# meyer-lab/cmtf-pls

Hardware: AMD Instinct MI355X
Metric: nipals_iters_per_sec (higher is better)
Workload: dtype f32

## Files before the change

cmtf_pls_amd/csrc/rank1.hip:

```cpp
#include "common.hpp"
#include <atomic>

namespace cmtfpls {

constexpr int kTile = 16;
constexpr int kMaxTiles = 256;
constexpr int kMaxSteps = 48;

struct Rank1Ctl {
  int done;
  int final_buf;
  int steps_used;
  int last_step;
  double pad[6];
};
__host__ __device__ __forceinline__ size_t rank1_ctl_bytes(int nt) {
  return sizeof(Rank1Ctl) + ((size_t)(kMaxSteps + 2) * nt + 2 * (size_t)nt * nt) * sizeof(double);
}
__device__ __forceinline__ double* ctl_trace(Rank1Ctl* c, int nt, int step) { return reinterpret_cast<double*>(c + 1) + (size_t)step * nt; }
__device__ __forceinline__ double* ctl_fro(Rank1Ctl* c, int nt, int which) {
  return reinterpret_cast<double*>(c + 1) + (size_t)(kMaxSteps + 2) * nt + (size_t)which * nt * nt;
}

__device__ __forceinline__ double pow2_scale_from_trace(const double* parts, int nt, double* tr_out) {
// ... 6 lines not shown
  return ldexp(1.0, -e);
}

typedef double d4r_t __attribute__((ext_vector_type(4)));

__global__ __launch_bounds__(kTile* kTile) void syrk_step_kernel(const double* __restrict__ M, int n, int k, int ld,
                                                                double* __restrict__ C, Rank1Ctl* __restrict__ ctl,
                                                                int step, int out_buf, double* __restrict__ C_keep) {
  __shared__ double red[4][kTile * kTile];
  __shared__ double diag[kTile];
  __shared__ double s_scale;
  __shared__ int s_done;
  __shared__ double fsum[4];
  __shared__ double tr_s[kMaxTiles];
  const int tx = threadIdx.x, ty = threadIdx.y, tid = ty * kTile + tx;
  const int lane = tid & 63, wv = tid >> 6, ri = lane & 15, kq = lane >> 4;
  const int nt = (n + kTile - 1) / kTile;
  const int i0 = blockIdx.y * kTile, j0 = blockIdx.x * kTile;

  constexpr int KC = 128, KW = 8;
  const bool ra = (i0 + ri) < n, rb = (j0 + ri) < n;
  const double* __restrict__ rowa = M + (int64_t)(ra ? i0 + ri : 0) * ld;
  const double* __restrict__ rowb = M + (int64_t)(rb ? j0 + ri : 0) * ld;
  const int cl = 32 * wv + KW * kq;
  double a[KW], b[KW];
#pragma unroll
  for (int s2 = 0; s2 < KW; ++s2) {
    const int c = cl + s2;
    const int cc = (c < k) ? c : 0;
    a[s2] = rowa[cc];
    b[s2] = rowb[cc];
  }

  double fro_in = 0.0;
  if (step >= 1) {
    int zero = 0;
    asm volatile("" : "+v"(zero));
    const int last_in = (&ctl->last_step)[zero];
    const int done_in = (&ctl->done)[zero] | ((last_in >= 0 && last_in < step) ? 1 : 0);
    const double* fp = ctl_fro(ctl, nt, (step - 1) & 1);
    const double trv = ctl_trace(ctl, nt, step - 1)[(tid < nt) ? tid : 0];
    double f = fp[(tid < nt * nt) ? tid : 0];
    if (tid < nt) tr_s[tid] = trv;
    if (tid >= nt * nt) f = 0.0;
    for (int i = tid + kTile * kTile; i < nt * nt; i += kTile * kTile) f += fp[i];
    f = wave_sum(f);
    if ((tid & 63) == 0) fsum[tid >> 6] = f;
    if (tid == 0) s_done = done_in;
    __syncthreads();
    fro_in = ((fsum[0] + fsum[1]) + fsum[2]) + fsum[3];
  }
  if (tid == 0) {
    int done = 0;
    double scale = 1.0;
    if (step == 0) {
      if (blockIdx.x == 0 && blockIdx.y == 0) { ctl->done = 0; ctl->final_buf = -1; ctl->steps_used = 0; ctl->last_step = -1; }
    } else {
      done = s_done;
      if (!done) {
        double tr1;
        scale = pow2_scale_from_trace(tr_s, nt, &tr1);
        const double rho = fro_in / (tr1 * tr1);
        const bool rank_one_in = !(tr1 > 0.0) || rho >= 1.0 - 1e-13;
        const bool rank_one_out = rho >= 1.0 - 1e-7;
        if (blockIdx.x == 0 && blockIdx.y == 0) {
          if (rank_one_in) { ctl->done = 1; ctl->final_buf = out_buf ^ 1; }
          else {
            ctl->steps_used = step;
            if (rank_one_out) { ctl->last_step = step; ctl->final_buf = out_buf; }
          }
        }
        if (rank_one_in) done = 1;
      }
    }
    s_scale = scale;
    s_done = done;
  }
  __syncthreads();
  if (s_done) return;
  const double scale = s_scale;

  d4r_t acc = d4r_t{0.0, 0.0, 0.0, 0.0};
  for (int kk = 0; kk < k; kk += KC) {
    if (kk > 0) {
#pragma unroll
      for (int s2 = 0; s2 < KW; ++s2) {
        const int c = kk + cl + s2;
        const int cc = (c < k) ? c : 0;
        a[s2] = rowa[cc];
        b[s2] = rowb[cc];
      }
    }
#pragma unroll
    for (int s2 = 0; s2 < KW; ++s2) {
      const bool cok = (kk + cl + s2) < k;
      const double av = (ra && cok) ? a[s2] : 0.0;
      const double bv = (rb && cok) ? b[s2] : 0.0;
      acc = __builtin_amdgcn_mfma_f64_16x16x4f64(av, bv, acc, 0, 0, 0);
    }
  }
#pragma unroll
  for (int e = 0; e < 4; ++e) red[wv][(kq + 4 * e) * kTile + ri] = acc[e];
  __syncthreads();
  double cacc = ((red[0][tid] + red[1][tid]) + red[2][tid]) + red[3][tid];
  cacc *= scale * scale;
  const bool inside = (i0 + ty < n && j0 + tx < n);
  if (inside) C[(int64_t)(i0 + ty) * n + (j0 + tx)] = cacc;
  if (inside && C_keep) C_keep[(int64_t)(i0 + ty) * n + (j0 + tx)] = cacc;
  {
    double sq = inside ? cacc * cacc : 0.0;
    sq = wave_sum(sq);
    if ((tid & 63) == 0) fsum[tid >> 6] = sq;
    __syncthreads();
    if (tid == 0) ctl_fro(ctl, nt, step & 1)[blockIdx.y * nt + blockIdx.x] = ((fsum[0] + fsum[1]) + fsum[2]) + fsum[3];
  }
  if (blockIdx.x == blockIdx.y) {
    if (tx == ty) diag[tx] = (i0 + ty < n) ? cacc : 0.0;
    __syncthreads();
    if (tid == 0) {
      double t = 0.0;
      for (int l = 0; l < kTile; ++l) t += diag[l];
      ctl_trace(ctl, nt, step)[blockIdx.x] = t;
    }
  }
}

constexpr unsigned long long kChainEmpty = ~0ull;
constexpr int kChainMaxSteps = 31;
constexpr int kChainSpin = 1 << 15;

__device__ __forceinline__ double chain_ld(const double* p) {
  return __longlong_as_double((long long)__hip_atomic_load(reinterpret_cast<const unsigned long long*>(p), __ATOMIC_RELAXED, __HIP_MEMORY_SCOPE_AGENT));
}
__device__ __forceinline__ void chain_st(double* p, double v) {
  unsigned long long b = (unsigned long long)__double_as_longlong(v);
  if (b == kChainEmpty) b = 0x7FF8000000000000ull;
  __hip_atomic_store(reinterpret_cast<unsigned long long*>(p), b, __ATOMIC_RELAXED, __HIP_MEMORY_SCOPE_AGENT);
}
__device__ __forceinline__ bool chain_empty(double v) { return (unsigned long long)__double_as_longlong(v) == kChainEmpty; }

__global__ __launch_bounds__(256) void chain_preset_kernel(unsigned long long* __restrict__ p, int64_t n) {
  for (int64_t i = (int64_t)blockIdx.x * 256 + threadIdx.x; i < n; i += (int64_t)gridDim.x * 256) p[i] = kChainEmpty;
}

#ifdef CMTFPLS_CHAIN_PROFILE
__device__ unsigned long long g_chain_prof[1024];
#define CHAIN_STAMP(slot) do { if (first_wg && tid == 0 && step < 32) g_chain_prof[step * 8 + (slot)] = __builtin_amdgcn_s_memrealtime(); } while (0)
#define CHAIN_COUNT(slot, v) do { if (first_wg && tid == 0 && step < 32) g_chain_prof[step * 8 + (slot)] = (unsigned long long)(v); } while (0)
#else
#define CHAIN_STAMP(slot) do { } while (0)
#define CHAIN_COUNT(slot, v) do { } while (0)
#endif

__global__ __launch_bounds__(kTile* kTile) void syrk_chain_kernel(const double* __restrict__ M0, int n, int k0,
                                                                 double* gbufs, double* trs, double* fros, double* gave_up,
                                                                 Rank1Ctl* __restrict__ ctl, int n_squarings) {
  constexpr int KC = 128, KW = 8, LDP = KC + 2;
  __shared__ __attribute__((aligned(16))) double pan[2][kTile][LDP];
  __shared__ double red[2][4][kTile * kTile];
  __shared__ double diag[2][kTile];
  __shared__ double fsum[2][4];
  __shared__ double cfro[2][4];
  __shared__ double ctr[2][kTile];
  __shared__ int cdead[2];
  const int tx = threadIdx.x, ty = threadIdx.y, tid = ty * kTile + tx;
  const int lane = tid & 63, wv = tid >> 6, ri = lane & 15, kq = lane >> 4;
  const int nt = (n + kTile - 1) / kTile, nt2 = nt * nt;
  const int i0 = blockIdx.y * kTile, j0 = blockIdx.x * kTile;
  const bool first_wg = blockIdx.x == 0 && blockIdx.y == 0;
  const bool ra = (i0 + ri) < n, rb = (j0 + ri) < n;
  const int cl = 32 * wv + KW * kq;
  const int64_t nn = (int64_t)n * n;
  const double qnan = __longlong_as_double(0x7FF8000000000000ll);
  bool dead = false;
  if (first_wg && tid == 0) { ctl->done = 0; ctl->final_buf = -1; ctl->steps_used = 0; ctl->last_step = -1; }
  if (tid < 2) cdead[tid] = 0;
  int last_step = -1;
  for (int step = 0; step <= n_squarings; ++step) {
    if (last_step >= 0) break;
    const int par = step & 1;
    const double* __restrict__ M = step == 0 ? M0 : gbufs + (int64_t)(step - 1) * nn;
    const int k = step == 0 ? k0 : n, ld = k;
    double* C = gbufs + (int64_t)step * nn;
    double a[KW], b[KW];
    double scale = 1.0;
    bool input_is_result = false;
    d4r_t acc = d4r_t{0.0, 0.0, 0.0, 0.0};
    CHAIN_STAMP(0);
    for (int kk = 0; kk < k; kk += KC) {
      if (step == 0) {
        const double* __restrict__ rowa = M + (int64_t)(ra ? i0 + ri : 0) * ld;
        const double* __restrict__ rowb = M + (int64_t)(rb ? j0 + ri : 0) * ld;
#pragma unroll
        for (int s2 = 0; s2 < KW; ++s2) {
          const int c = kk + cl + s2;
          const int cc = (c < k) ? c : 0;
          a[s2] = rowa[cc];
          b[s2] = rowb[cc];
        }
      } else {
        double va[8], vb[8], trv = 0.0, f = 0.0;
        const bool first_chunk = kk == 0;
        const double* tp = trs + (int64_t)(step - 1) * nt;
        const double* fp = fros + (int64_t)(step - 1) * nt2;
        unsigned offa[8], offb[8];
#pragma unroll
        for (int i = 0; i < 8; ++i) {
          const int e = tid + 256 * i, r = e >> 7, c = kk + (e & 127);
          const int cc = (c < k) ? c : 0;
          const int rra = (i0 + r < n) ? i0 + r : 0, rrb = (j0 + r < n) ? j0 + r : 0;
          offa[i] = (unsigned)(rra * ld + cc);
          offb[i] = (unsigned)(rrb * ld + cc);
        }
        int spins = 0;
        for (;;) {
          bool ok = true;
#pragma unroll
          for (int i = 0; i < 8; ++i) {
            va[i] = chain_ld(M + offa[i]);
            vb[i] = chain_ld(M + offb[i]);
          }
          if (first_chunk) {
            f = chain_ld(fp + ((tid < nt2) ? tid : 0));
            ok = !chain_empty(f);
            if (wv == 0) {
              trv = chain_ld(tp + ((lane < nt) ? lane : 0));
              ok = ok && !chain_empty(trv);
            }
          }
#pragma unroll
          for (int i = 0; i < 8; ++i) ok = ok && !chain_empty(va[i]) && !chain_empty(vb[i]);
          if (dead || __all(ok)) break;
          if (++spins > kChainSpin) {
            dead = true;
            if (lane == 0) chain_st(gave_up, 1.0);
            break;
          }
        }
        CHAIN_STAMP(1);
        CHAIN_COUNT(7, spins);
        if (kk > 0) __syncthreads();
#pragma unroll
        for (int i = 0; i < 8; ++i) {
          const int e = tid + 256 * i, r = e >> 7, c = e & 127;
          pan[0][r][c] = dead ? qnan : va[i];
          pan[1][r][c] = dead ? qnan : vb[i];
        }
        if (first_chunk) {
          const double fw = wave_sum((tid < nt2) ? f : 0.0);
          if (lane == 0) cfro[par][wv] = fw;
          if (wv == 0 && lane < nt) ctr[par][lane] = trv;
          if (dead && lane == 0) cdead[par] = 1;
        }
        __syncthreads();
        CHAIN_STAMP(2);
        if (first_chunk) {
          const double fro_in = ((cfro[par][0] + cfro[par][1]) + cfro[par][2]) + cfro[par][3];
          double tr1 = 0.0;
          for (int i = 0; i < nt; ++i) tr1 += ctr[par][i];
          if ((tr1 > 0.0) && isfinite(tr1)) {
            int e;
            frexp(tr1, &e);
            scale = ldexp(1.0, -e);
          }
          const bool gone = cdead[par] != 0;
          const double rho = fro_in / (tr1 * tr1);
          const bool rank_one_in = !gone && (!(tr1 > 0.0) || rho >= 1.0 - 1e-13);
          const bool rank_one_out = !gone && rho >= 1.0 - 1e-7;
          if (first_wg && tid == 0) {
            if (rank_one_in) { ctl->done = 1; ctl->final_buf = step - 1; }
            else {
              ctl->steps_used = step;
              if (rank_one_out) { ctl->last_step = step; ctl->final_buf = step; }
            }
          }
          if (rank_one_in) { input_is_result = true; break; }
          if (rank_one_out) last_step = step;
        }
#pragma unroll
        for (int s2 = 0; s2 < KW; ++s2) {
          a[s2] = pan[0][ri][cl + s2];
          b[s2] = pan[1][ri][cl + s2];
        }
      }
#pragma unroll
      for (int s2 = 0; s2 < KW; ++s2) {
        const bool cok = (kk + cl + s2) < k;
        const double av = (ra && cok) ? a[s2] : 0.0;
        const double bv = (rb && cok) ? b[s2] : 0.0;
        acc = __builtin_amdgcn_mfma_f64_16x16x4f64(av, bv, acc, 0, 0, 0);
      }
    }
    if (input_is_result) break;
    CHAIN_STAMP(3);
#pragma unroll
    for (int e = 0; e < 4; ++e) red[par][wv][(kq + 4 * e) * kTile + ri] = acc[e];
    __syncthreads();
    CHAIN_STAMP(4);
    double cacc = ((red[par][0][tid] + red[par][1][tid]) + red[par][2][tid]) + red[par][3][tid];
    cacc *= scale * scale;
    const bool inside = (i0 + ty < n && j0 + tx < n);
    if (inside) chain_st(C + (int64_t)(i0 + ty) * n + (j0 + tx), cacc);
    CHAIN_STAMP(5);
    double sq = inside ? cacc * cacc : 0.0;
    sq = wave_sum(sq);
    if ((tid & 63) == 0) fsum[par][tid >> 6] = sq;
    if (blockIdx.x == blockIdx.y && tx == ty) diag[par][tx] = (i0 + ty < n) ? cacc : 0.0;
    __syncthreads();
    if (tid == 0) {
      chain_st(fros + (int64_t)step * nt2 + blockIdx.y * nt + blockIdx.x, ((fsum[par][0] + fsum[par][1]) + fsum[par][2]) + fsum[par][3]);
      if (blockIdx.x == blockIdx.y) {
        double t = 0.0;
        for (int l = 0; l < kTile; ++l) t += diag[par][l];
        chain_st(trs + (int64_t)step * nt + blockIdx.x, t);
      }
    }
    CHAIN_STAMP(6);
  }
}

__global__ __launch_bounds__(256) void transpose_kernel(const double* __restrict__ Z, int A, int B, double* __restrict__ Zt) {
  const int64_t idx = (int64_t)blockIdx.x * 256 + threadIdx.x;
  if (idx >= (int64_t)A * B) return;
  const int b = (int)(idx / A), a = (int)(idx % A);
  Zt[idx] = Z[(int64_t)a * B + b];
}

__global__ __launch_bounds__(256) void rank1_seed_xy_kernel(const double* __restrict__ M, int n, int k,
                                                           const double* __restrict__ gbase, int64_t gstride,
                                                           const double* __restrict__ G0,
                                                           const Rank1Ctl* __restrict__ ctl, int last_buf, int ny_blocks,
                                                           double* __restrict__ y, double* __restrict__ x) {
  extern __shared__ double seed[];
  __shared__ double red[16];
  __shared__ double rsum[8][33];
  __shared__ double bestv[4];
  __shared__ int besti[4];
  const int fb = (ctl->final_buf >= 0) ? ctl->final_buf : last_buf;
  const double* G = gbase + (int64_t)fb * gstride;
  double bv = -1.0;
  int bi = 0;
  for (int i = threadIdx.x; i < n; i += 256) {
    const double d = G[(int64_t)i * n + i];
    if (d > bv) { bv = d; bi = i; }
  }
#pragma unroll
  for (int m = 32; m > 0; m >>= 1) {
    const double ov = __shfl_xor(bv, m, 64);
    const int oi = __shfl_xor(bi, m, 64);
    if (ov > bv || (ov == bv && oi < bi)) { bv = ov; bi = oi; }
  }
  if ((threadIdx.x & 63) == 0) { bestv[threadIdx.x >> 6] = bv; besti[threadIdx.x >> 6] = bi; }
  __syncthreads();
  bv = bestv[0];
  bi = besti[0];
  for (int w = 1; w < 4; ++w)
    if (bestv[w] > bv || (bestv[w] == bv && besti[w] < bi)) { bv = bestv[w]; bi = besti[w]; }
  double ss = 0.0;
  for (int i = threadIdx.x; i < n; i += 256) {
    const double g = G[(int64_t)bi * n + i];
    seed[i] = g;
    ss = fma(g, g, ss);
  }
  const double nrm = sqrt(block_sum(ss, red));
  for (int i = threadIdx.x; i < n; i += 256) seed[i] = seed[i] / nrm;
  __syncthreads();
  if ((int)blockIdx.x >= ny_blocks) {
    const int j = ((int)blockIdx.x - ny_blocks) * 4 + (threadIdx.x >> 6);
    const int lane = threadIdx.x & 63;
    if (j < n) {
      double s = 0.0;
      for (int i = lane; i < n; i += 64) s = fma(G0[(int64_t)j * n + i], seed[i], s);
      s = wave_sum(s);
      if (lane == 0) x[j] = s;
    }
    return;
  }
  const int cx = threadIdx.x & 31, ry = threadIdx.x >> 5;
  const int c = blockIdx.x * 32 + cx;
  double s = 0.0;
  if (c < k)
    for (int j = ry; j < n; j += 8) s = fma(M[(int64_t)j * k + c], seed[j], s);
  rsum[ry][cx] = s;
  __syncthreads();
  if (ry == 0 && c < k) {
    double tot = 0.0;
#pragma unroll
    for (int g = 0; g < 8; ++g) tot += rsum[g][cx];
    y[c] = tot;
  }
}

__device__ __forceinline__ void rank1_write_info(double* __restrict__ info, const Rank1Ctl* __restrict__ ctl, const double* gave) {
  if (!info) return;
  if (gave && !chain_empty(chain_ld(gave))) { info[0] = 0.0; info[1] = -1.0; return; }
  info[0] = (ctl->done || ctl->last_step >= 0) ? 1.0 : 0.0;
  info[1] = (double)ctl->steps_used;
}

__device__ __forceinline__ void rank1_final_body(const double* x, const double* y,
                                                 int n, int k, int x_is_A, const Rank1Ctl* __restrict__ ctl,
                                                 double* __restrict__ wA, double* __restrict__ wB,
                                                 double* __restrict__ sigma, double* __restrict__ info, const double* gave) {
  __shared__ double red[2][16];
  __shared__ double bestv[16];
  __shared__ int besti[16];
  double sx = 0.0, sy = 0.0;
  for (int i = threadIdx.x; i < n; i += 1024) sx = fma(x[i], x[i], sx);
  for (int i = threadIdx.x; i < k; i += 1024) sy = fma(y[i], y[i], sy);
  const double nx = sqrt(block_sum(sx, red[0]));
  const double ny = sqrt(block_sum(sy, red[1]));
  const double* vb = x_is_A ? y : x;
  const int nb = x_is_A ? k : n;
  double bv = -1.0;
  int bi = 0;
  for (int i = threadIdx.x; i < nb; i += 1024) {
    const double d = fabs(vb[i]);
    if (d > bv) { bv = d; bi = i; }
  }
#pragma unroll
  for (int m = 32; m > 0; m >>= 1) {
    const double ov = __shfl_xor(bv, m, 64);
    const int oi = __shfl_xor(bi, m, 64);
    if (ov > bv || (ov == bv && oi < bi)) { bv = ov; bi = oi; }
  }
  if ((threadIdx.x & 63) == 0) { bestv[threadIdx.x >> 6] = bv; besti[threadIdx.x >> 6] = bi; }
  __syncthreads();
  bv = bestv[0];
  bi = besti[0];
  for (int w = 1; w < 16; ++w)
    if (bestv[w] > bv || (bestv[w] == bv && besti[w] < bi)) { bv = bestv[w]; bi = besti[w]; }
  const bool gv = gave && !chain_empty(chain_ld(gave));
  const double sgn = gv ? __longlong_as_double(0x7FF8000000000000ll) : ((vb[bi] < 0.0) ? -1.0 : 1.0);
  double* ox = x_is_A ? wA : wB;
  double* oy = x_is_A ? wB : wA;
  for (int i = threadIdx.x; i < n; i += 1024) ox[i] = sgn * (x[i] / nx);
  for (int i = threadIdx.x; i < k; i += 1024) oy[i] = sgn * (y[i] / ny);
  if (threadIdx.x == 0) {
    if (sigma) sigma[0] = nx / ny;
    rank1_write_info(info, ctl, gave);
  }
}

__global__ __launch_bounds__(1024) void rank1_final_kernel(const double* __restrict__ x, const double* __restrict__ y,
                                                          int n, int k, int x_is_A, const Rank1Ctl* __restrict__ ctl,
                                                          double* __restrict__ wA, double* __restrict__ wB,
                                                          double* __restrict__ sigma, double* __restrict__ info, const double* gave) {
  rank1_final_body(x, y, n, k, x_is_A, ctl, wA, wB, sigma, info, gave);
}

__global__ __launch_bounds__(1024) void rank1_final_score_kernel(const double* __restrict__ x, const double* __restrict__ y,
                                                                int n, int k, int x_is_A, const Rank1Ctl* __restrict__ ctl,
                                                                double* __restrict__ wA, double* __restrict__ wB,
                                                                double* __restrict__ info, const double* __restrict__ S, int A, int B,
                                                                double* __restrict__ t, const double* gave) {
  extern __shared__ double lds[];
  __shared__ double red[2][16];
  __shared__ double bestv[16];
  __shared__ int besti[16];
  double* sA = lds;
  double* sB = lds + ((A + 1) & ~1);
  double sx = 0.0, sy = 0.0;
  for (int i = threadIdx.x; i < n; i += 1024) sx = fma(x[i], x[i], sx);
  for (int i = threadIdx.x; i < k; i += 1024) sy = fma(y[i], y[i], sy);
  const double nx = sqrt(block_sum(sx, red[0]));
  const double ny = sqrt(block_sum(sy, red[1]));
  const double* vb = x_is_A ? y : x;
  const int nb = x_is_A ? k : n;
  double bv = -1.0;
  int bi = 0;
  for (int i = threadIdx.x; i < nb; i += 1024) {
    const double d = fabs(vb[i]);
    if (d > bv) { bv = d; bi = i; }
  }
#pragma unroll
  for (int m = 32; m > 0; m >>= 1) {
    const double ov = __shfl_xor(bv, m, 64);
    const int oi = __shfl_xor(bi, m, 64);
    if (ov > bv || (ov == bv && oi < bi)) { bv = ov; bi = oi; }
  }
  if ((threadIdx.x & 63) == 0) { bestv[threadIdx.x >> 6] = bv; besti[threadIdx.x >> 6] = bi; }
  __syncthreads();
  bv = bestv[0];
  bi = besti[0];
  for (int w = 1; w < 16; ++w)
    if (bestv[w] > bv || (bestv[w] == bv && besti[w] < bi)) { bv = bestv[w]; bi = besti[w]; }
  const bool gv = gave && !chain_empty(chain_ld(gave));
  const double sgn = gv ? __longlong_as_double(0x7FF8000000000000ll) : ((vb[bi] < 0.0) ? -1.0 : 1.0);
  double* lx = x_is_A ? sA : sB;
  double* ly = x_is_A ? sB : sA;
  double* ox = x_is_A ? wA : wB;
  double* oy = x_is_A ? wB : wA;
  const bool store = blockIdx.x == 0;
  for (int i = threadIdx.x; i < n; i += 1024) {
    const double v = sgn * (x[i] / nx);
    lx[i] = v;
    if (store) ox[i] = v;
  }
  for (int i = threadIdx.x; i < k; i += 1024) {
    const double v = sgn * (y[i] / ny);
    ly[i] = v;
    if (store) oy[i] = v;
  }
  if (store && threadIdx.x == 0) rank1_write_info(info, ctl, gave);
  __syncthreads();
  using VT = Pack<double, 2>;
  const int64_t P = (int64_t)A * B;
  const int64_t step = (int64_t)1024 * 2;
  const double* __restrict__ xr = S + (int64_t)blockIdx.x * P;
  KronWalk w((int64_t)threadIdx.x * 2, step, B);
  double acc = 0.0;
  int64_t c = (int64_t)threadIdx.x * 2;
  constexpr int UN = 4;
  for (; c + (UN - 1) * step < P; c += UN * step) {
    VT xs[UN];
#pragma unroll
    for (int u = 0; u < UN; ++u) xs[u] = ld_stream(reinterpret_cast<const VT*>(xr + c + u * step));
#pragma unroll
    for (int u = 0; u < UN; ++u) {
      double d = 0.0;
      d = fma(xs[u].e[0], sB[w.k], d);
      d = fma(xs[u].e[1], sB[w.k + 1], d);
      acc = fma(sA[w.j], d, acc);
      w.next();
    }
  }
  for (; c < P; c += step) {
    const VT xv = ld_stream(reinterpret_cast<const VT*>(xr + c));
    double d = 0.0;
    d = fma(xv.e[0], sB[w.k], d);
    d = fma(xv.e[1], sB[w.k + 1], d);
    acc = fma(sA[w.j], d, acc);
    w.next();
  }
  acc = block_sum(acc, red[0]);
  if (threadIdx.x == 0) t[blockIdx.x] = acc;
}

static inline size_t align_up(size_t x, size_t a) { return (x + a - 1) / a * a; }

static std::atomic<int> g_chain_on{1};

static int chain_slots() {
  static int slots = 0;
  if (slots == 0) {
    int dev = 0, cus = 0;
    if (hipGetDevice(&dev) != hipSuccess || hipDeviceGetAttribute(&cus, hipDeviceAttributeMultiprocessorCount, dev) != hipSuccess || cus <= 0) cus = 256;
    slots = 2 * cus;
  }
  return slots;
}

}

using namespace cmtfpls;

extern "C" {

size_t cmtfpls_rank1_workspace_bytes(int A, int B) {
  if (A <= 0 || B <= 0) return 0;
  const size_t n = (size_t)(A < B ? A : B), k = (size_t)(A < B ? B : A);
  const size_t nt = (n + kTile - 1) / kTile;
  const size_t chain = nt * nt <= 256 ? align_up(((size_t)(kChainMaxSteps + 1) * (n * n + nt + nt * nt) + 1) * sizeof(double), 256) : 0;
  return align_up(rank1_ctl_bytes((int)nt), 256) + 3 * align_up(n * n * sizeof(double), 256) +
         align_up((size_t)A * B * sizeof(double), 256) + align_up(n * sizeof(double), 256) + align_up(k * sizeof(double), 256) + chain;
}

static int rank1_run(const double* Z, int A, int B, double* wA, double* wB, double* sigma, double* info,
                     int n_squarings, void* ws, size_t ws_bytes, void* stream, const double* S, int M, double* tq, bool allow_chain = true);

int cmtfpls_rank1_f64(const double* Z, int A, int B, double* wA, double* wB, double* sigma, double* info,
                      int n_squarings, void* ws, size_t ws_bytes, void* stream) {
  return rank1_run(Z, A, B, wA, wB, sigma, info, n_squarings, ws, ws_bytes, stream, nullptr, 0, nullptr);
}

#ifdef CMTFPLS_CHAIN_PROFILE
int cmtfpls_debug_chain_prof(unsigned long long* out) { return (int)hipMemcpyFromSymbol(out, HIP_SYMBOL(g_chain_prof), sizeof(unsigned long long) * 1024); }
#endif
void cmtfpls_rank1_chain_enable(int on) { g_chain_on.store((on == 1 || on == 2) ? on : 0, std::memory_order_relaxed); }
int cmtfpls_rank1_chain_enabled(void) { return g_chain_on.load(std::memory_order_relaxed); }

int cmtfpls_rank1_launches_f64(const double* Z, int A, int B, double* wA, double* wB, double* sigma, double* info,
                               int n_squarings, void* ws, size_t ws_bytes, void* stream) {
  return rank1_run(Z, A, B, wA, wB, sigma, info, n_squarings, ws, ws_bytes, stream, nullptr, 0, nullptr, false);
}

int cmtfpls_rank1_score_f64(const double* Z, int A, int B, double* wA, double* wB, double* info, int n_squarings,
                            const double* S, int M, double* tq, void* ws, size_t ws_bytes, void* stream) {
  if (!S || !tq || M <= 0) { set_error("rank1_score: bad argument"); return CMTFPLS_EINVAL; }
  const int64_t P = (int64_t)A * B;
  if (M > 64 || P < 8192 || (B % 2) != 0 || ((size_t)(((A + 1) & ~1) + B) * sizeof(double)) > 60 * 1024 ||
      (reinterpret_cast<uintptr_t>(S) & 15) != 0) {
    int rc = cmtfpls_rank1_f64(Z, A, B, wA, wB, nullptr, info, n_squarings, ws, ws_bytes, stream);
    if (rc == CMTFPLS_OK) rc = cmtfpls_score_s_f64(S, M, A, B, wA, wB, tq, stream);
    return rc;
  }
  return rank1_run(Z, A, B, wA, wB, nullptr, info, n_squarings, ws, ws_bytes, stream, S, M, tq);
}

static int rank1_run(const double* Z, int A, int B, double* wA, double* wB, double* sigma, double* info,
                     int n_squarings, void* ws, size_t ws_bytes, void* stream, const double* S, int M, double* tq, bool allow_chain) {
  if (!Z || !wA || !wB || A <= 0 || B <= 0) { set_error("rank1: bad argument"); return CMTFPLS_EINVAL; }
  const int n = A < B ? A : B, k = A < B ? B : A;
  if (n > kTile * kMaxTiles) { set_error("rank1: min(A, B) > 4096 unsupported"); return CMTFPLS_EUNSUPPORTED; }
  if ((size_t)n * sizeof(double) > 64 * 1024) { set_error("rank1: seed exceeds the LDS"); return CMTFPLS_EUNSUPPORTED; }
  if (n_squarings < 1) n_squarings = 1;
  if (n_squarings > kMaxSteps) n_squarings = kMaxSteps;
  if (!ws || ws_bytes < cmtfpls_rank1_workspace_bytes(A, B)) { set_error("rank1: workspace too small"); return CMTFPLS_EWORKSPACE; }
  hipStream_t st = (hipStream_t)stream;
  char* p = static_cast<char*>(ws);
  Rank1Ctl* ctl = reinterpret_cast<Rank1Ctl*>(p);
  p += align_up(rank1_ctl_bytes((n + kTile - 1) / kTile), 256);
  double* buf0 = reinterpret_cast<double*>(p);
  p += align_up((size_t)n * n * sizeof(double), 256);
  double* buf1 = reinterpret_cast<double*>(p);
  p += align_up((size_t)n * n * sizeof(double), 256);
  double* g0keep = reinterpret_cast<double*>(p);
  p += align_up((size_t)n * n * sizeof(double), 256);
  double* Zt = reinterpret_cast<double*>(p);
  p += align_up((size_t)A * B * sizeof(double), 256);
  double* xv = reinterpret_cast<double*>(p);
  p += align_up((size_t)n * sizeof(double), 256);
  double* yv = reinterpret_cast<double*>(p);
  p += align_up((size_t)k * sizeof(double), 256);
  double* chain_region = reinterpret_cast<double*>(p);

  const double* M0 = Z;
  if (A > B) {
    const int64_t tot = (int64_t)A * B;
    hipLaunchKernelGGL(transpose_kernel, dim3((unsigned)((tot + 255) / 256)), dim3(256), 0, st, Z, A, B, Zt);
    M0 = Zt;
  }
  const int nt = (n + kTile - 1) / kTile;
  const dim3 grid(nt, nt), block(kTile, kTile);
  const int ny_blocks = (k + 31) / 32;
  const double* gave = nullptr;
  if (allow_chain && g_chain_on.load(std::memory_order_relaxed) && nt * nt <= 256 && nt * nt <= chain_slots() && n_squarings <= kChainMaxSteps) {
    const size_t nn = (size_t)n * n, steps = (size_t)n_squarings + 1;
    double* gbufs = chain_region;
    double* trs = gbufs + steps * nn;
    double* fros = trs + steps * nt;
    double* gave_up = fros + steps * (size_t)nt * nt;
    gave = gave_up;
    const int64_t words = (int64_t)(steps * (nn + nt + (size_t)nt * nt) + 1);
    hipLaunchKernelGGL(chain_preset_kernel, dim3((unsigned)((words + 2047) / 2048)), dim3(256), 0, st, reinterpret_cast<unsigned long long*>(chain_region), words);
    const dim3 cgrid(nt, (g_chain_on.load(std::memory_order_relaxed) == 2 && nt > 1) ? nt - 1 : nt);
    hipLaunchKernelGGL(syrk_chain_kernel, cgrid, block, 0, st, M0, n, k, gbufs, trs, fros, gave_up, ctl, n_squarings);
    hipLaunchKernelGGL(rank1_seed_xy_kernel, dim3(ny_blocks + (n + 3) / 4), dim3(256), (size_t)n * sizeof(double), st,
                       M0, n, k, gbufs, (int64_t)nn, gbufs, ctl, n_squarings, ny_blocks, yv, xv);
  } else {
    hipLaunchKernelGGL(syrk_step_kernel, grid, block, 0, st, M0, n, k, k, buf0, ctl, 0, 0, g0keep);
    for (int s = 1; s <= n_squarings; ++s) {
      const double* in = (s & 1) ? buf0 : buf1;
      double* out = (s & 1) ? buf1 : buf0;
      hipLaunchKernelGGL(syrk_step_kernel, grid, block, 0, st, in, n, n, n, out, ctl, s, s & 1, (double*)nullptr);
    }
    hipLaunchKernelGGL(rank1_seed_xy_kernel, dim3(ny_blocks + (n + 3) / 4), dim3(256), (size_t)n * sizeof(double), st,
                       M0, n, k, buf0, (int64_t)(buf1 - buf0), g0keep, ctl, n_squarings & 1, ny_blocks, yv, xv);
  }
  if (S) {
    const size_t lds = (size_t)(((A + 1) & ~1) + B) * sizeof(double);
    hipLaunchKernelGGL(rank1_final_score_kernel, dim3((unsigned)M), dim3(1024), lds, st, xv, yv, n, k, (A <= B) ? 1 : 0, ctl, wA, wB, info,
                       S, A, B, tq, gave);
    return check_launch("rank1_score");
  }
  hipLaunchKernelGGL(rank1_final_kernel, dim3(1), dim3(1024), 0, st, xv, yv, n, k, (A <= B) ? 1 : 0, ctl, wA, wB, sigma, info, gave);
  return check_launch("rank1");
}

}
```

cmtf_pls_amd/fitrun.py:

```python
from __future__ import annotations

import math
from typing import Dict, List, Optional

import numpy as np
import torch

from .fitrun_xcov import XcovMixin
from .state import BlockState, FitState, split_trailing, validate_limits


class FitRun(XcovMixin):

    def __init__(self, eng: NipalsEngine, Xs: List[torch.Tensor], Y: torch.Tensor, n_components: int, coupled: bool,
                 algorithm: str = "direct", owned: Optional[List[bool]] = None, allow_raw: bool = True):
        be, comm = eng.be, eng.comm
        Xs = list(Xs)
        owned = [True] * len(Xs) if owned is None else list(owned)
        if algorithm not in ("direct", "xcov"):
            raise ValueError("algorithm must be 'direct' or 'xcov'")
        self.algorithm_requested = self.algorithm = algorithm
        self.notes: List[str] = []
        validate_limits([tuple(X.shape) for X in Xs], n_components)
        self.eng, self.Xs, self.Y, self.R, self.coupled = eng, Xs, Y, n_components, coupled
# ... 538 lines not shown

    def _inner_regression(self, a: int, extra: Optional[torch.Tensor] = None):
        be, comm = self.eng.be, self.eng.comm
        k = a + 1
        Ta = self.T[:, :k]
        G = be.gram_tn(Ta, Ta)
        g = be.gram_tn(Ta, self.u)
        if comm.sharded:
            packed = torch.cat([G.reshape(-1), g.reshape(-1)] + ([extra.reshape(-1)] if extra is not None else []))
            comm.allreduce(packed)
            G, g = packed[: k * k].view(k, k), packed[k * k: k * k + k]
            extra = packed[k * k + k:] if extra is not None else None
        b_dev = be.normal_solve(G, g.reshape(-1), out=self.b_dev[:k])
        self.coef_dev[:k, a].copy_(b_dev)
        self._G_last = G
        return b_dev, extra

    def _finish_fused(self, a: int) -> None:
        be, comm = self.eng.be, self.eng.comm
        k = a + 1
        b_dev, _ = self._inner_regression(a)
        ssqy = be.y_deflate(self.Y, self.T, k, b_dev, self.q)
        ssqs = []
        self._z_ready = False
        if k < self.R:
            q0 = self.qbuf[0]
            q0.zero_()
            q0[0] = 1.0
            ready = True
            for b, blk in enumerate(self.blocks):
                s_b = be.deflate_contract_yq(self.X2[b], blk.A, blk.B, self.t, self.wA[b], self.wB[b], self.Y, q0,
                                             blk.has_miss, out=self.Zs[b])
                if s_b is None:
                    s_b = be.deflate(self.X2[b], blk.A, blk.B, self.t, self.wA[b], self.wB[b])
                    ready = False
                ssqs.append(s_b)
            self._z_ready = ready
        else:
            for b, blk in enumerate(self.blocks):
                ssqs.append(be.deflate(self.X2[b], blk.A, blk.B, self.t, self.wA[b], self.wB[b]))
        self._log_ssq(a, ssqs, ssqy)

    def _log_ssq(self, a: int, ssqs, ssqy) -> None:
        for b in range(len(self.blocks)):
            self.ssq_log[a, b].copy_(ssqs[b].reshape(()))
        self.ssq_log[a, len(self.blocks)].copy_(ssqy.reshape(()))

    def _store_component(self, a: int) -> None:
        self.T[:, a].copy_(self.t)
        self.U[:, a].copy_(self.u)
        self.Q[:, a].copy_(self.q)
        self._store_loadings(a)

    def _store_loadings(self, a: int) -> None:
        for b, blk in enumerate(self.blocks):
            if len(blk.shape) == 2:
                blk.loadings[0][:, a].copy_(self.wB[b])
            elif len(blk.shape) == 3:
                blk.loadings[0][:, a].copy_(self.wA[b])
                blk.loadings[1][:, a].copy_(self.wB[b])
            else:
                for m, d in enumerate(blk.shape[1:]):
                    blk.loadings[m][:, a].copy_(self.fac[b][m, :d])

    def result(self) -> FitState:
        if getattr(self, "_state", None) is not None:
            return self._state
        nb = len(self.blocks)
        nowrite = self.algorithm == "xcov" and getattr(self, "_nowrite", False)
        for b, ssq in getattr(self, "_ssq0_dev", {}).items():
            self.blocks[b].ssq0 = float(ssq.item())
        self.eng.comm.allreduce(self.ssq_log)
        parts = [self.coef_dev.reshape(-1), self.ssq_log.reshape(-1)]
        if nowrite:
            self.eng.comm.allreduce(self.dot_log)
            parts.append(self.dot_log.reshape(-1))
        host = torch.cat(parts).cpu().numpy()
        R = self.R
        self.coef[...] = host[: R * R].reshape(R, R)
        ssq = host[R * R: R * R + R * (nb + 1)].reshape(R, nb + 1).copy()
        if nowrite:
            dots = host[R * R + R * (nb + 1):].reshape(R, 1 + nb)
            for b, blk in enumerate(self.blocks):
                run = blk.ssq0
                for a in range(len(self.n_iter)):
                    run = run - 2.0 * dots[a, 1 + b] + dots[a, 0]
                    ssq[a, b] = run
        for a in range(len(self.n_iter)):
            for b, blk in enumerate(self.blocks):
                blk.r2x[a] = 1.0 - ssq[a, b] / blk.ssq0
            self.r2y[a] = 1.0 - ssq[a, nb] / self.ssqy0
        self._state = FitState(coupled=self.coupled, n_components=self.R, blocks=self.blocks, T=self.T, U=self.U, Q=self.Q,
                               coef=self.coef, r2y=self.r2y, y_mean=self.y_mean, n_iter=self.n_iter,
                               n_samples_total=self.n_total, report=self.build_report())
        return self._state

    def build_report(self) -> Dict[str, object]:
        eng, comm, nb = self.eng, self.eng.comm, len(self.blocks)
        rep: Dict[str, object] = {
            "form": "regular", "algorithm_requested": self.algorithm_requested, "algorithm": self.algorithm,
            "shapes": [tuple(b.shape) for b in self.blocks], "storage": [str(b.dtype).replace("torch.", "") for b in self.blocks],
            "missing": [bool(b.has_miss) for b in self.blocks], "responses": self.M,
            "sharded": bool(comm.sharded), "world": int(comm.world),
            "graphs": bool(self.use_graphs and self._graphs), "graph_error": self._graph_error,
            "collectives_in_graph": self._collectives_captured is True,
            "backend": getattr(eng.be, "name", type(eng.be).__name__),
        }
        if self.algorithm == "direct":
            rep["y_side"] = "fused into the sweeps" if self._fused else "separate launches"
            if not self._fused and self.M > 64:
                self.notes.append("Y side not fused into the sweeps: more than 64 responses")
            rep["x_passes_per_iteration"] = "2 reads"
            rep["x_passes_per_component"] = ("1 read + write (deflation fused with the next contraction)" if self._fused
                                             else "1 read + write (deflation)")
            rep["x_copy"] = "centred private copy"
        else:
            nowrite = bool(getattr(self, "_nowrite", False))
            one_read = nowrite and bool(getattr(self, "_one_read", False))
            any_miss = any(b.has_miss for b in self.blocks)
            rep["x_copy"] = "none: the caller's uncentred tensor is read in place" if self.raw else "centred private copy"
            rep["raw"] = bool(self.raw)
            rep["x_written"] = not nowrite
            rep["s_carried"] = bool(self._s_carry)
            rep["s_build"] = ("per component (missing values)" if any_miss else "first component only") + \
                             (f", {(self.M + 63) // 64} response tiles of <= 64" if self.M > 64 else "") + \
                             (", [Y, Y * rowscale] in one pass" if any(x is not None for x in self.S12) else "")
            rep["one_read"] = one_read
            rep["stats_with_s"] = bool(getattr(self, "_stats_with_s", False))
            if nowrite:
                rep["x_passes_per_component"] = ("1 read (largest block); 2 reads (other blocks)" if one_read and nb > 1 else
                                                 "1 read" if one_read else "2 reads")
            elif any_miss and nb == 1 and getattr(self, "_deflate_build_ok", True) and self.S12[0] is not None and eng.opt.xcov_deflate_build:
                rep["x_passes_per_component"] = "1 read + 1 read + write (deflation inside the rebuild of S)"
            elif any_miss:
                rep["x_passes_per_component"] = "1 read + write (score + deflation) + S rebuild reads"
            else:
                rep["x_passes_per_component"] = "1 read + 1 read + write"
            rep["pipelined"] = bool(getattr(self, "_pipelined", False))
            if rep["pipelined"]:
                rep["pipeline"] = dict(self.pipeline_stats)
            if not rep["pipelined"] and eng.opt.xcov_pipeline:
                why = ("graph replay requested" if self.use_graphs else "more than 64 responses" if self.M > 64 else
                       "a block of order > 3 or a backend without the single-call iteration")
                self.notes.append("inner loop on S not pipelined: " + why)
            if self.algorithm_requested == "xcov" and not self.raw and eng.opt.xcov_raw and not any_miss and not any("uncentred" in n for n in self.notes):
                self.notes.append("uncentred xcov form declined: " + ("more than 64 components" if self.R > 64 else
                                                                      "f32 matrix precision or a backend without its kernels"))
            if nowrite and eng.opt.xcov_one_read and self.R > 1 and not one_read:
                self.notes.append("one read per component declined: the row does not fit the registers of 1..16 workgroups "
                                  "(rows of 2048..131072 f32 -- 262144 when the last mode divides 4096 -- / 1024..131072 f64 elements, "
                                  "last mode a multiple of 4 / 2)")
        rep["rank1_one_launch_chain"] = bool(getattr(eng.be, "rank1_chain_side", 0)) and any(
            len(blk.shape) == 3 and min(blk.A, blk.B) <= int(getattr(eng.be, "rank1_chain_side", 0)) for blk in self.blocks)
        rep["declined"] = list(self.notes)
        return rep
```

Measured before the change: 769.8.

## Fold transpose, seed/xy projection and finalisation into the single chain kernel

Result: no change. 769.6 (median of 6 runs) (-0.0%).

```diff
diff --git a/cmtf_pls_amd/csrc/rank1.hip b/cmtf_pls_amd/csrc/rank1.hip
--- a/cmtf_pls_amd/csrc/rank1.hip
+++ b/cmtf_pls_amd/csrc/rank1.hip
@@ -182,9 +182,27 @@
 #define CHAIN_COUNT(slot, v) do { } while (0)
 #endif
 
-__global__ __launch_bounds__(kTile* kTile) void syrk_chain_kernel(const double* __restrict__ M0, int n, int k0,
+__device__ __forceinline__ double chain_wait(const double* p, bool active, bool& dead, bool lane0, double* gave_up) {
+  double v = 0.0;
+  int spins = 0;
+  for (;;) {
+    if (active) v = chain_ld(p);
+    if (dead || __all(!active || !chain_empty(v))) break;
+    if (++spins > kChainSpin) {
+      dead = true;
+      if (lane0) chain_st(gave_up, 1.0);
+      break;
+    }
+  }
+  return dead ? __longlong_as_double(0x7FF8000000000000ll) : v;
+}
+
+__global__ __launch_bounds__(kTile* kTile) void syrk_chain_kernel(const double* __restrict__ M0, int n, int k0, int trans,
                                                                  double* gbufs, double* trs, double* fros, double* gave_up,
-                                                                 Rank1Ctl* __restrict__ ctl, int n_squarings) {
+                                                                 unsigned long long* arrive, Rank1Ctl* __restrict__ ctl,
+                                                                 int n_squarings, double* xx, double* yy, int x_is_A,
+                                                                 double* __restrict__ wA, double* __restrict__ wB,
+                                                                 double* __restrict__ sigma, double* __restrict__ info) {
   constexpr int KC = 128, KW = 8, LDP = KC + 2;
   __shared__ __attribute__((aligned(16))) double pan[2][kTile][LDP];
   __shared__ double red[2][4][kTile * kTile];
@@ -193,6 +211,7 @@
   __shared__ double cfro[2][4];
   __shared__ double ctr[2][kTile];
   __shared__ int cdead[2];
+  __shared__ int anydead, s_last;
   const int tx = threadIdx.x, ty = threadIdx.y, tid = ty * kTile + tx;
   const int lane = tid & 63, wv = tid >> 6, ri = lane & 15, kq = lane >> 4;
   const int nt = (n + kTile - 1) / kTile, nt2 = nt * nt;
@@ -205,7 +224,9 @@
   bool dead = false;
   if (first_wg && tid == 0) { ctl->done = 0; ctl->final_buf = -1; ctl->steps_used = 0; ctl->last_step = -1; }
   if (tid < 2) cdead[tid] = 0;
+  if (tid == 0) anydead = 0;
   int last_step = -1;
+  int steps_used = 0, final_step = -1;
   for (int step = 0; step <= n_squarings; ++step) {
     if (last_step >= 0) break;
     const int par = step & 1;
@@ -219,14 +240,13 @@
     CHAIN_STAMP(0);
     for (int kk = 0; kk < k; kk += KC) {
       if (step == 0) {
-        const double* __restrict__ rowa = M + (int64_t)(ra ? i0 + ri : 0) * ld;
-        const double* __restrict__ rowb = M + (int64_t)(rb ? j0 + ri : 0) * ld;
+        const int rowa = ra ? i0 + ri : 0, rowb = rb ? j0 + ri : 0;
 #pragma unroll
         for (int s2 = 0; s2 < KW; ++s2) {
           const int c = kk + cl + s2;
           const int cc = (c < k) ? c : 0;
-          a[s2] = rowa[cc];
-          b[s2] = rowb[cc];
+          a[s2] = trans ? M[(int64_t)cc * n + rowa] : M[(int64_t)rowa * ld + cc];
+          b[s2] = trans ? M[(int64_t)cc * n + rowb] : M[(int64_t)rowb * ld + cc];
         }
       } else {
         double va[8], vb[8], trv = 0.0, f = 0.0;
@@ -304,7 +324,8 @@
               if (rank_one_out) { ctl->last_step = step; ctl->final_buf = step; }
             }
           }
-          if (rank_one_in) { input_is_result = true; break; }
+          if (rank_one_in) { input_is_result = true; final_step = step - 1; break; }
+          steps_used = step;
           if (rank_one_out) last_step = step;
         }
 #pragma unroll
@@ -347,6 +368,200 @@
     }
     CHAIN_STAMP(6);
   }
+
+  const int fb = final_step >= 0 ? final_step : (last_step >= 0 ? last_step : n_squarings);
+  const double* Gf = gbufs + (int64_t)fb * nn;
+  const int nwg = gridDim.x * gridDim.y, wg = blockIdx.y * gridDim.x + blockIdx.x;
+  const int ny_blocks = (k0 + 31) / 32, nroles = ny_blocks + (n + 3) / 4;
+  const bool lane0 = lane == 0;
+  double* seed = &pan[0][0][0];
+  double(*rsum)[33] = reinterpret_cast<double(*)[33]>(&pan[0][0][0] + 256);
+  __shared__ double ered[2][16];
+  __shared__ double ebv[16];
+  __shared__ int ebi[16];
+  __syncthreads();
+  if (wg < nroles) {
+    const bool act = tid < n;
+    const double d = chain_wait(Gf + (act ? (int64_t)tid * n + tid : 0), act, dead, lane0, gave_up);
+    double bv = -1.0;
+    int bi = 0;
+    if (act && d > bv) { bv = d; bi = tid; }
+#pragma unroll
+    for (int m = 32; m > 0; m >>= 1) {
+      const double ov = __shfl_xor(bv, m, 64);
+      const int oi = __shfl_xor(bi, m, 64);
+      if (ov > bv || (ov == bv && oi < bi)) { bv = ov; bi = oi; }
+    }
+    if (lane0) { ebv[wv] = bv; ebi[wv] = bi; }
+    __syncthreads();
+    bv = ebv[0];
+    bi = ebi[0];
+    for (int w = 1; w < 4; ++w)
+      if (ebv[w] > bv || (ebv[w] == bv && ebi[w] < bi)) { bv = ebv[w]; bi = ebi[w]; }
+    const double g = chain_wait(Gf + (int64_t)bi * n + (act ? tid : 0), act, dead, lane0, gave_up);
+    if (act) seed[tid] = g;
+    double ss = act ? fma(g, g, 0.0) : 0.0;
+    ss = wave_sum(ss);
+    if (lane0) ered[0][wv] = ss;
+    __syncthreads();
+    double nsq = 0.0;
+    for (int w = 0; w < 4; ++w) nsq += ered[0][w];
+    const double nrm = sqrt(nsq);
+    if (act) seed[tid] = seed[tid] / nrm;
+    __syncthreads();
+    for (int role = wg; role < nroles; role += nwg) {
+      if (role >= ny_blocks) {
+        const int j = (role - ny_blocks) * 4 + wv;
+        if (j < n) {
+          double s = 0.0;
+          for (int c0 = 0; c0 < n; c0 += 64) {
+            const int i = c0 + lane;
+            const double v = chain_wait(gbufs + (int64_t)j * n + (i < n ? i : 0), i < n, dead, lane0, gave_up);
+            if (i < n) s = fma(v, seed[i], s);
+          }
+          s = wave_sum(s);
+          if (lane0) chain_st(xx + j, s);
+        }
+      } else {
+        const int cx = tid & 31, ry = tid >> 5;
+        const int c = role * 32 + cx;
+        double s = 0.0;
+        if (c < k0)
+          for (int j = ry; j < n; j += 8) s = fma(trans ? M0[(int64_t)c * n + j] : M0[(int64_t)j * k0 + c], seed[j], s);
+        rsum[ry][cx] = s;
+        __syncthreads();
+        if (ry == 0 && c < k0) {
+          double tot = 0.0;
+#pragma unroll
+          for (int g8 = 0; g8 < 8; ++g8) tot += rsum[g8][cx];
+          chain_st(yy + c, tot);
+        }
+        __syncthreads();
+      }
+    }
+  }
+
+  if (dead && lane0) anydead = 1;
+  __syncthreads();
+  if (tid == 0) {
+    const unsigned long long inc = 1ull + (anydead ? (1ull << 32) : 0ull);
+    const unsigned long long cnt = __hip_atomic_fetch_add(arrive, inc, __ATOMIC_RELAXED, __HIP_MEMORY_SCOPE_AGENT) + 1ull + inc;
+    s_last = (cnt & 0xFFFFFFFFull) == (unsigned long long)nwg ? ((cnt >> 32) ? 2 : 1) : 0;
+  }
+  __syncthreads();
+  if (!s_last) return;
+
+  const int k = k0;
+  double* xl = &pan[0][0][0];
+  double* yl = xl + n;
+  const bool in_lds = n + k <= 2 * kTile * LDP;
+  for (int c0 = 0; c0 < n; c0 += 256) {
+    const double v = chain_wait(xx + (c0 + tid < n ? c0 + tid : 0), c0 + tid < n, dead, lane0, gave_up);
+    if (in_lds && c0 + tid < n) xl[c0 + tid] = v;
+  }
+  for (int c0 = 0; c0 < k; c0 += 256) {
+    const double v = chain_wait(yy + (c0 + tid < k ? c0 + tid : 0), c0 + tid < k, dead, lane0, gave_up);
+    if (in_lds && c0 + tid < k) yl[c0 + tid] = v;
+  }
+  if (dead && lane0) anydead = 1;
+  __syncthreads();
+  const bool gv = s_last == 2 || anydead;
+  auto ldx = [&](int i) { return in_lds ? xl[i] : chain_ld(xx + i); };
+  auto ldy = [&](int i) { return in_lds ? yl[i] : chain_ld(yy + i); };
+#pragma unroll
+  for (int v = 0; v < 4; ++v) {
+    const int V = tid + 256 * v;
+    double sx = 0.0, sy = 0.0;
+    for (int i = V; i < n; i += 1024) { const double e = ldx(i); sx = fma(e, e, sx); }
+    for (int i = V; i < k; i += 1024) { const double e = ldy(i); sy = fma(e, e, sy); }
+    sx = wave_sum(sx);
+    sy = wave_sum(sy);
+    if (lane0) { ered[0][wv + 4 * v] = sx; ered[1][wv + 4 * v] = sy; }
+  }
+  __syncthreads();
+  double nx = 0.0, ny = 0.0;
+  for (int w = 0; w < 16; ++w) nx += ered[0][w];
+  for (int w = 0; w < 16; ++w) ny += ered[1][w];
+  nx = sqrt(nx);
+  ny = sqrt(ny);
+  const int nb = x_is_A ? k : n;
+  auto ldb = [&](int i) { return x_is_A ? ldy(i) : ldx(i); };
+#pragma unroll
+  for (int v = 0; v < 4; ++v) {
+    const int V = tid + 256 * v;
+    double bv = -1.0;
+    int bi = 0;
+    for (int i = V; i < nb; i += 1024) {
+      const double d = fabs(ldb(i));
+      if (d > bv) { bv = d; bi = i; }
+    }
+#pragma unroll
+    for (int m = 32; m > 0; m >>= 1) {
+      const double ov = __shfl_xor(bv, m, 64);
+      const int oi = __shfl_xor(bi, m, 64);
+      if (ov > bv || (ov == bv && oi < bi)) { bv = ov; bi = oi; }
+    }
+    if (lane0) { ebv[wv + 4 * v] = bv; ebi[wv + 4 * v] = bi; }
+  }
+  __syncthreads();
+  double bv = ebv[0];
+  int bi = ebi[0];
+  for (int w = 1; w < 16; ++w)
+    if (ebv[w] > bv || (ebv[w] == bv && ebi[w] < bi)) { bv = ebv[w]; bi = ebi[w]; }
+  const double sgn = gv ? qnan : ((ldb(bi) < 0.0) ? -1.0 : 1.0);
+  double* ox = x_is_A ? wA : wB;
+  double* oy = x_is_A ? wB : wA;
+  for (int i = tid; i < n; i += 256) ox[i] = sgn * (ldx(i) / nx);
+  for (int i = tid; i < k; i += 256) oy[i] = sgn * (ldy(i) / ny);
+  if (tid == 0) {
+    if (sigma) sigma[0] = nx / ny;
+    if (info) {
+      if (gv) { info[0] = 0.0; info[1] = -1.0; }
+      else { info[0] = (final_step >= 0 || last_step >= 0) ? 1.0 : 0.0; info[1] = (double)steps_used; }
+    }
+  }
+}
+
+__global__ __launch_bounds__(1024) void rank1_score_rows_kernel(const double* __restrict__ wA, const double* __restrict__ wB,
+                                                               const double* __restrict__ S, int A, int B, double* __restrict__ t) {
+  extern __shared__ double lds[];
+  __shared__ double red[16];
+  double* sA = lds;
+  double* sB = lds + ((A + 1) & ~1);
+  for (int i = threadIdx.x; i < A; i += 1024) sA[i] = wA[i];
+  for (int i = threadIdx.x; i < B; i += 1024) sB[i] = wB[i];
+  __syncthreads();
+  using VT = Pack<double, 2>;
+  const int64_t P = (int64_t)A * B;
+  const int64_t step = (int64_t)1024 * 2;
+  const double* __restrict__ xr = S + (int64_t)blockIdx.x * P;
+  KronWalk w((int64_t)threadIdx.x * 2, step, B);
+  double acc = 0.0;
+  int64_t c = (int64_t)threadIdx.x * 2;
+  constexpr int UN = 4;
+  for (; c + (UN - 1) * step < P; c += UN * step) {
+    VT xs[UN];
+#pragma unroll
+    for (int u = 0; u < UN; ++u) xs[u] = ld_stream(reinterpret_cast<const VT*>(xr + c + u * step));
+#pragma unroll
+    for (int u = 0; u < UN; ++u) {
+      double d = 0.0;
+      d = fma(xs[u].e[0], sB[w.k], d);
+      d = fma(xs[u].e[1], sB[w.k + 1], d);
+      acc = fma(sA[w.j], d, acc);
+      w.next();
+    }
+  }
+  for (; c < P; c += step) {
+    const VT xv = ld_stream(reinterpret_cast<const VT*>(xr + c));
+    double d = 0.0;
+    d = fma(xv.e[0], sB[w.k], d);
+    d = fma(xv.e[1], sB[w.k + 1], d);
+    acc = fma(sA[w.j], d, acc);
+    w.next();
+  }
+  acc = block_sum(acc, red);
+  if (threadIdx.x == 0) t[blockIdx.x] = acc;
 }
 
 __global__ __launch_bounds__(256) void transpose_kernel(const double* __restrict__ Z, int A, int B, double* __restrict__ Zt) {
@@ -572,13 +787,20 @@
 static std::atomic<int> g_chain_on{1};
 
 static int chain_slots() {
-  static int slots = 0;
-  if (slots == 0) {
-    int dev = 0, cus = 0;
-    if (hipGetDevice(&dev) != hipSuccess || hipDeviceGetAttribute(&cus, hipDeviceAttributeMultiprocessorCount, dev) != hipSuccess || cus <= 0) cus = 256;
-    slots = 2 * cus;
-  }
-  return slots;
+  constexpr int kDevs = 64;
+  static std::atomic<int> slots[kDevs];
+  int dev = 0;
+  if (hipGetDevice(&dev) != hipSuccess || dev < 0 || dev >= kDevs) return 0;
+  int s = slots[dev].load(std::memory_order_relaxed);
+  if (s == 0) {
+    int cus = 0, per_cu = 0;
+    if (hipDeviceGetAttribute(&cus, hipDeviceAttributeMultiprocessorCount, dev) != hipSuccess || cus <= 0 ||
+        hipOccupancyMaxActiveBlocksPerMultiprocessor(&per_cu, syrk_chain_kernel, kTile * kTile, 0) != hipSuccess || per_cu < 0)
+      return 0;
+    s = per_cu * cus;
+    slots[dev].store(s > 0 ? s : -1, std::memory_order_relaxed);
+  }
+  return s > 0 ? s : 0;
 }
 
 }
@@ -591,7 +813,7 @@
   if (A <= 0 || B <= 0) return 0;
   const size_t n = (size_t)(A < B ? A : B), k = (size_t)(A < B ? B : A);
   const size_t nt = (n + kTile - 1) / kTile;
-  const size_t chain = nt * nt <= 256 ? align_up(((size_t)(kChainMaxSteps + 1) * (n * n + nt + nt * nt) + 1) * sizeof(double), 256) : 0;
+  const size_t chain = nt * nt <= 256 ? align_up(((size_t)(kChainMaxSteps + 1) * (n * n + nt + nt * nt) + 2) * sizeof(double), 256) : 0;
   return align_up(rank1_ctl_bytes((int)nt), 256) + 3 * align_up(n * n * sizeof(double), 256) +
          align_up((size_t)A * B * sizeof(double), 256) + align_up(n * sizeof(double), 256) + align_up(k * sizeof(double), 256) + chain;
 }
@@ -655,46 +877,50 @@
   p += align_up((size_t)k * sizeof(double), 256);
   double* chain_region = reinterpret_cast<double*>(p);
 
-  const double* M0 = Z;
-  if (A > B) {
-    const int64_t tot = (int64_t)A * B;
-    hipLaunchKernelGGL(transpose_kernel, dim3((unsigned)((tot + 255) / 256)), dim3(256), 0, st, Z, A, B, Zt);
-    M0 = Zt;
-  }
   const int nt = (n + kTile - 1) / kTile;
   const dim3 grid(nt, nt), block(kTile, kTile);
   const int ny_blocks = (k + 31) / 32;
-  const double* gave = nullptr;
+  const int x_is_A = (A <= B) ? 1 : 0;
   if (allow_chain && g_chain_on.load(std::memory_order_relaxed) && nt * nt <= 256 && nt * nt <= chain_slots() && n_squarings <= kChainMaxSteps) {
     const size_t nn = (size_t)n * n, steps = (size_t)n_squarings + 1;
     double* gbufs = chain_region;
     double* trs = gbufs + steps * nn;
     double* fros = trs + steps * nt;
     double* gave_up = fros + steps * (size_t)nt * nt;
-    gave = gave_up;
-    const int64_t words = (int64_t)(steps * (nn + nt + (size_t)nt * nt) + 1);
-    hipLaunchKernelGGL(chain_preset_kernel, dim3((unsigned)((words + 2047) / 2048)), dim3(256), 0, st, reinterpret_cast<unsigned long long*>(chain_region), words);
+    unsigned long long* arrive = reinterpret_cast<unsigned long long*>(gave_up + 1);
+    const int64_t words = (int64_t)(chain_region - xv) + (int64_t)(steps * (nn + nt + (size_t)nt * nt) + 2);
+    hipLaunchKernelGGL(chain_preset_kernel, dim3((unsigned)((words + 2047) / 2048)), dim3(256), 0, st, reinterpret_cast<unsigned long long*>(xv), words);
     const dim3 cgrid(nt, (g_chain_on.load(std::memory_order_relaxed) == 2 && nt > 1) ? nt - 1 : nt);
-    hipLaunchKernelGGL(syrk_chain_kernel, cgrid, block, 0, st, M0, n, k, gbufs, trs, fros, gave_up, ctl, n_squarings);
-    hipLaunchKernelGGL(rank1_seed_xy_kernel, dim3(ny_blocks + (n + 3) / 4), dim3(256), (size_t)n * sizeof(double), st,
-                       M0, n, k, gbufs, (int64_t)nn, gbufs, ctl, n_squarings, ny_blocks, yv, xv);
-  } else {
-    hipLaunchKernelGGL(syrk_step_kernel, grid, block, 0, st, M0, n, k, k, buf0, ctl, 0, 0, g0keep);
-    for (int s = 1; s <= n_squarings; ++s) {
-      const double* in = (s & 1) ? buf0 : buf1;
-      double* out = (s & 1) ? buf1 : buf0;
-      hipLaunchKernelGGL(syrk_step_kernel, grid, block, 0, st, in, n, n, n, out, ctl, s, s & 1, (double*)nullptr);
-    }
-    hipLaunchKernelGGL(rank1_seed_xy_kernel, dim3(ny_blocks + (n + 3) / 4), dim3(256), (size_t)n * sizeof(double), st,
-                       M0, n, k, buf0, (int64_t)(buf1 - buf0), g0keep, ctl, n_squarings & 1, ny_blocks, yv, xv);
-  }
+    hipLaunchKernelGGL(syrk_chain_kernel, cgrid, block, 0, st, Z, n, k, (A > B) ? 1 : 0, gbufs, trs, fros, gave_up, arrive, ctl,
+                       n_squarings, xv, yv, x_is_A, wA, wB, S ? nullptr : sigma, info);
+    if (S) {
+      const size_t lds = (size_t)(((A + 1) & ~1) + B) * sizeof(double);
+      hipLaunchKernelGGL(rank1_score_rows_kernel, dim3((unsigned)M), dim3(1024), lds, st, wA, wB, S, A, B, tq);
+      return check_launch("rank1_score");
+    }
+    return check_launch("rank1");
+  }
+  const double* M0 = Z;
+  if (A > B) {
+    const int64_t tot = (int64_t)A * B;
+    hipLaunchKernelGGL(transpose_kernel, dim3((unsigned)((tot + 255) / 256)), dim3(256), 0, st, Z, A, B, Zt);
+    M0 = Zt;
+  }
+  hipLaunchKernelGGL(syrk_step_kernel, grid, block, 0, st, M0, n, k, k, buf0, ctl, 0, 0, g0keep);
+  for (int s = 1; s <= n_squarings; ++s) {
+    const double* in = (s & 1) ? buf0 : buf1;
+    double* out = (s & 1) ? buf1 : buf0;
+    hipLaunchKernelGGL(syrk_step_kernel, grid, block, 0, st, in, n, n, n, out, ctl, s, s & 1, (double*)nullptr);
+  }
+  hipLaunchKernelGGL(rank1_seed_xy_kernel, dim3(ny_blocks + (n + 3) / 4), dim3(256), (size_t)n * sizeof(double), st,
+                     M0, n, k, buf0, (int64_t)(buf1 - buf0), g0keep, ctl, n_squarings & 1, ny_blocks, yv, xv);
   if (S) {
     const size_t lds = (size_t)(((A + 1) & ~1) + B) * sizeof(double);
-    hipLaunchKernelGGL(rank1_final_score_kernel, dim3((unsigned)M), dim3(1024), lds, st, xv, yv, n, k, (A <= B) ? 1 : 0, ctl, wA, wB, info,
-                       S, A, B, tq, gave);
+    hipLaunchKernelGGL(rank1_final_score_kernel, dim3((unsigned)M), dim3(1024), lds, st, xv, yv, n, k, x_is_A, ctl, wA, wB, info,
+                       S, A, B, tq, nullptr);
     return check_launch("rank1_score");
   }
-  hipLaunchKernelGGL(rank1_final_kernel, dim3(1), dim3(1024), 0, st, xv, yv, n, k, (A <= B) ? 1 : 0, ctl, wA, wB, sigma, info, gave);
+  hipLaunchKernelGGL(rank1_final_kernel, dim3(1), dim3(1024), 0, st, xv, yv, n, k, x_is_A, ctl, wA, wB, sigma, info, nullptr);
   return check_launch("rank1");
 }
 
diff --git a/cmtf_pls_amd/fitrun.py b/cmtf_pls_amd/fitrun.py
--- a/cmtf_pls_amd/fitrun.py
+++ b/cmtf_pls_amd/fitrun.py
@@ -714,5 +714,6 @@
                                   "last mode a multiple of 4 / 2)")
         rep["rank1_one_launch_chain"] = bool(getattr(eng.be, "rank1_chain_side", 0)) and any(
             len(blk.shape) == 3 and min(blk.A, blk.B) <= int(getattr(eng.be, "rank1_chain_side", 0)) for blk in self.blocks)
+        rep["rank1_form"] = "one launch" if rep["rank1_one_launch_chain"] else "launch per squaring"
         rep["declined"] = list(self.notes)
         return rep
```
